# ArtRand/cPecan-signal

Hardware: AMD Instinct MI355X
Metric: banded fwd-bwd Gcells/s (higher is better)
Workload: dtype f64

## Files before the change

cpecan-signal_amd/csrc/asm/gen_sweeps.py:

```python
#!/usr/bin/env python3
import os
import struct
import sys

from emit import Emitter, Neg, Pool, S, V

L = 3
P = 64 * L

LAYER_BYTES = 2 * 64 * 16
OFF_FXY = 64 * 16
OFF_PY = L * LAYER_BYTES
PY2_X2 = os.environ.get("CPECAN_ASM_PY2", "x2") == "x2"
ROW_BYTES = L * LAYER_BYTES + 1024 + (512 if PY2_X2 else 1024)
ROW_DOUBLES = ROW_BYTES // 8
assert L == 3
TRACK_ROW_BYTES = 20 * 8
NCONST = 18

A_ITEMS, A_TRACKBASE, A_PLANWIN, A_PLANCTL, A_PLANOFF, A_EVENTS, A_MODELS, A_TRACK = 0, 8, 16, 24, 32, 40, 48, 56
A_RING, A_RINGDOUBLES, A_STATES, A_CTX, A_CTXBYTES, A_COEF, A_NITEMS, A_WINDOW = 64, 72, 80, 88, 96, 104, 112, 116
A_RINGD, A_MAXWIN, A_SCRATCH, A_SCRATCHBYTES, A_LOGTHR, A_MODELSTRIDE, ARGS_BYTES = 120, 124, 128, 136, 144, 152, 168
A_MASKTAB = 160
I_LX, I_LY, I_YOFF, I_DIAGBASE, I_MODEL, I_RAGGEDL, I_RAGGEDR, ITEM_BYTES = 0, 8, 24, 48, 112, 116, 120, 128
# ... 7 lines not shown
CTX_X = L * 9 * 1024
CTX_S = CTX_X + 2 * L * 1536
CTX_BYTES = CTX_S + 256

LDS_COEF = 0
LDS_EV = 512
EVN = 256
LDS_ROWS = LDS_EV + ((2 * EVN + L) * 16 + 63) // 64 * 64
ROWN = 64
LDS_F_BYTES = LDS_ROWS + ROWN * TRACK_ROW_BYTES
LDS_PX = 512
PXN = 64
LDS_RF = LDS_PX + PXN * 16
LDS_RF_XY_T = LDS_RF
LDS_B_BYTES = LDS_RF + L * 1024

MAX_WIDTH = 158
BLOCK = 64

ABLATE = set(os.environ.get("CPECAN_ASM_ABLATE", "").split())

LOG2E_F32 = 0x3FB8AA3B
LN2_F32 = 0x3F317218


def dbits(x):
    return struct.unpack("<Q", struct.pack("<d", x))[0]


class Kernel(Emitter):
# ... 103 lines not shown
            self.valu("v_fma_f64", dst, dst, "-0.5", K)
        self.pool.give(*t1s)

    def ladd_front_group(self, pairs, free=()):
        p = self.pool
        recs = [[p.take(2), p.take(2), p.take(2), None, None] for _ in pairs]
        for (x, y), r in zip(pairs, recs):
            self.valu("v_max_f64", r[0], x, y)
        for (x, y), r in zip(pairs, recs):
            self.valu("v_min_f64", r[1], x, y)
        p.give(*free)
        for r in recs:
            self.add(r[2], r[0], Neg(r[1]))
        return recs

    def s_mov64_lit(self, dst, value):
        self.salu("s_mov_b32", dst.lo, "0x%x" % (value & 0xFFFFFFFF))
        self.salu("s_mov_b32", dst.hi, "0x%x" % (value >> 32))

    def add64(self, dst, a, b_lo, b_hi=0):
        self.salu("s_add_u32", dst.lo, a.lo, b_lo)
        self.salu("s_addc_u32", dst.hi, a.hi, b_hi)

    def pc_of(self, dst, label):
        here = self.newlabel("pc")
        self.salu("s_getpc_b64", dst)
        self.label(here)
        self.salu("s_add_u32", dst.lo, dst.lo, "%s-%s" % (label, here))
        self.salu("s_addc_u32", dst.hi, dst.hi, 0)

# ... 58 lines not shown
    sPlanRec = S(90, 2)
    lbl = lambda s: ".L_%s_%s" % (name, s)

    def load_store_masks(q):
        k.salu("s_lshl_b32", sT[0], sD, 6)
        k.salu("s_add_u32", sT[0], sT[0], 32)
        k.smem("s_load_dwordx4", S(sMaskS[q][0].i, 4), sMaskTab, sT[0])
        k.salu("s_add_u32", sT[0], sT[0], 16)
        if PY2_X2:
            k.smem("s_load_dwordx2", sMaskS[q][2], sMaskTab, sT[0])
            k.salu("s_add_u32", sT[0], sT[0], 8)
            k.smem("s_load_dwordx2", sMaskPy2[q], sMaskTab, sT[0])
        else:
            k.smem("s_load_dwordx2", sMaskS[q][2], sMaskTab, sT[0])

    def masked_store(mask, dwords, voff, data, off, gate=None):
        if "NOSTORE" in ABLATE or ("NOSTORE4" in ABLATE and dwords == 4) or ("NOSTORE2" in ABLATE and dwords == 2):
            return
        if "STOREALL" in ABLATE:
            if gate is None:
                k.gstore(dwords, voff, data, sRow0 if off < 4096 else sRow1, off % 4096)
            return
        if isinstance(mask, tuple):
            k.salu("s_or_b64", "exec", mask[0], mask[1])
        elif gate is None:
            k.salu("s_mov_b64", "exec", mask)
        else:
            k.salu("s_and_b64", "exec", mask, gate)
        if "EXECONLY" not in ABLATE:
            k.gstore(dwords, voff, data, sRow0 if off < 4096 else sRow1, off % 4096)
        k.salu("s_mov_b64", "exec", -1)
# ... 183 lines not shown
        k.salu("s_sub_u32", sD, sD, 1)
        k.lgkm = []
        k.salu("s_bitcmp1_b64", sStepMin, sD)
        if "NOEVENTS" not in ABLATE:
            k.branch("s_cbranch_scc1", lbl("leave%d" % p))
        k.label(lbl("left%d" % p))
        k.salu("s_bitcmp1_b64", sStepMax, sD)
        if "NOEVENTS" not in ABLATE:
            k.branch("s_cbranch_scc1", lbl("enter%d" % p))
        k.label(lbl("entered%d" % p))
        k.lgkm = pend
        k.salu("s_and_b32", sT[0], sD, sRingMask)
        k.salu("s_mul_i32", sT[0], sT[0], ROW_BYTES)
        k.add64(sRow0, sRing, sT[0])
        k.add64(sRow1, sRow0, 4096)

        def lower(j, w):
            return (Xm(q, j - 1), Xx(q, j - 1))[w] if j else R[q].sub(2 * w, 2)

        def middle(j, w):
            return (Xm(p, j - 1), Xx(p, j - 1), Xy(p, j - 1))[w] if j else R[p].sub(2 * w, 2)

        if "HALFPRIO" in ABLATE:
            k.salu("s_setprio", 2)
        aa, bb = [pool.take(2) for _ in range(L)], [pool.take(2) for _ in range(L)]
        for j in range(L):
            k.add(aa[j], lower(j, 0), C[j][CPXO])
        for j in range(L):
            k.add(bb[j], lower(j, 1), C[j][CPXE])
        recs = k.ladd_front_group(list(zip(aa, bb)), free=aa + bb)
# ... 61 lines not shown
        k.need_recs(recs)
        k.ladd_back_group(recs, [Xy(p, j) for j in range(L)])
        k.salu("s_bitcmp1_b64", sFull, sD)
        k.branch("s_cbranch_scc1", lbl("full%d" % p))
        k.label(lbl("fulled%d" % p))
        recs = k.ladd_front_group([(Xm(p, j), csum[j]) for j in range(L)], free=csum)
        k.ladd_rows(recs)
        k.ror64(R[p].sub(2, 2), Xx(p, L - 1))
        k.ror64(R[p].sub(4, 2), Xy(p, L - 1))
        k.need_recs(recs)
        k.ladd_back_group(recs, [Xm(p, j) for j in range(L)])
        masked_store(sMaskS[p][0], 4, vOff16, V(Xm(p, 0).i, 4), 0)
        k.ror64(R[p].sub(0, 2), Xm(p, L - 1))
        for j in range(1, L):
            masked_store(sMaskS[p][j], 4, vOff16, V(Xm(p, j).i, 4), j * LAYER_BYTES)
        k.salu("s_add_u32", sD, sD, 1)

    k.label(lbl("even"))
    step(0)
    state_after = list(k.lgkm)
    k.salu("s_cmp_gt_i32", sD, sTop)
    k.branch("s_cbranch_scc1", lbl("done"))
    k.label(lbl("odd"))
    k.vm = []
    step(1)
    k.salu("s_cmp_le_i32", sD, sStop)
    k.branch("s_cbranch_scc1", lbl("even"))
    k.salu("s_cmp_gt_i32", sD, sTop)
    k.branch("s_cbranch_scc1", lbl("done"))
    k.salu("s_swappc_b64", sRet, sStagePC)
    k.branch("s_branch", lbl("even"))

    for p in range(2):
        k.forget()
        k.label(lbl("full%d" % p))
        for j in range(L):
            masked_store(sMaskS[p][j], 4, vOff16, V(X[p][j].i + 4, 4), j * LAYER_BYTES + OFF_FXY)
        k.branch("s_branch", lbl("fulled%d" % p))
    for p in range(2):
        k.forget()
        k.label(lbl("leave%d" % p))
        k.salu("s_add_u32", sXmin, sXmin, 1)
        k.salu("s_lshl_b64", sBit, 1, sOutL)
        for j in range(L - 1):
            k.salu("s_cmp_eq_u32", sOutJ, j)
            k.branch("s_cbranch_scc1", lbl("leave%d_%d" % (p, j)))
        for j in reversed(range(L)):
            if j < L - 1:
                k.label(lbl("leave%d_%d" % (p, j)))
            k.salu("s_andn2_b64", sMask[j], sMask[j], sBit)
# ... 327 lines not shown
    sRow0, sRow1 = S(20, 2), S(22, 2)
    SM = [S(24 + 8 * q, 8) for q in range(3)]
    def SMm(q, j): return SM[q].sub(2 * j, 2)
    def SMxmin(q): return SM[q].sub(6)
    def SMxmax(q): return SM[q].sub(7)
    sB = [S(24 + i) for i in range(24)]
    def sBp(i): return S(24 + i, 2)
    sMaskTab, sTrack = S(48, 2), S(50, 2)
    sTMM, sTXM, sTYM, sTMY, sTYY = S(52, 2), S(54, 2), S(56, 2), S(58, 2), S(60, 2)
    s7p5, sNinf = S(62, 2), S(64, 2)
    sRf, sWtot, sCandKx, sCandFb, sState = S(66, 2), S(68, 2), S(70, 2), S(72, 2), S(74, 2)
    sA = [S(76 + i) for i in range(16)]
    def sAp(i): return S(76 + i, 2)
    sRet, sStagePC = S(92, 2), S(94, 2)
    sLm = [S(96 + 2 * j, 2) for j in range(L)]
    sCmp = [S(84 + 2 * j, 2) for j in range(L)]
    lbl = lambda s: ".L_%s_%s" % (name, s)

    k.label(name)
    if "PRIOB" in ABLATE:
        k.salu("s_setprio", 2)
    k.smem("s_load_dwordx4", S(24, 4), sArg, A_NITEMS)
    k.smem("s_load_dwordx2", sBp(4), sArg, A_PLANWIN)
    k.smem("s_load_dwordx2", sBp(6), sArg, A_STATES)
    k.smem("s_load_dwordx2", sBp(8), sArg, A_ITEMS)
    k.smem("s_load_dwordx2", sBp(10), sArg, A_LOGTHR)
    k.wait_lgkm()
    k.salu("s_cmp_ge_u32", sWg, sB[0])
    k.branch("s_cbranch_scc1", lbl("exit"))
    k.salu("s_mov_b32", sWindow, sB[1])
# ... 132 lines not shown
    k.salu("s_mov_b32", sNTot, 0)
    k.salu("s_mov_b32", sTd, sTop)
    k.valu("v_mov_b32_e32", vThr.lo, 0)
    k.valu("v_mov_b32_e32", vThr.hi, "0x7ff00000")
    k.salu("s_sub_u32", sRefCnt, sTop, sTpost0)
    k.salu("s_cmp_le_i32", sTop, sFrom)
    k.branch("s_cbranch_scc0", lbl("nodecode"))
    k.valu("v_mov_b32_e32", vThr.lo, vCthr.lo)
    k.valu("v_mov_b32_e32", vThr.hi, vCthr.hi)
    k.label(lbl("nodecode"))
    k.pc_of(sStagePC, lbl("stage"))
    k.wait_all()
    for h in range(2):
        k.rol64(RP.sub(2 * h, 2), PX[0].sub(2 * h, 2))
    def prefetch_terms(dreg, masks=None):
        k.salu("s_and_b32", sA[0], dreg, sRingMask)
        k.salu("s_mul_i32", sA[0], sA[0], ROW_BYTES)
        k.add64(sAp(4), sRing0, sA[0])
        for j in range(L):
            if masks is not None:
                k.salu("s_lshr_b64", sAp(8), masks[j], 8)
                k.salu("s_lshl_b64", sAp(10), masks[j], 56)
                k.salu("s_or_b64", sAp(8), sAp(8), sAp(10))
                k.salu("s_or_b64", "exec", sAp(8), masks[j])
            k.add64(sAp(2), sAp(4), j * LAYER_BYTES + OFF_FXY)
            k.salu("s_mov_b32", "m0", LDS_RF_XY_T + j * 1024)
            k.nop(1)
            k.gload_lds(vOff16, sAp(2))
        if masks is not None:
            k.salu("s_mov_b64", "exec", -1)

    prefetch_terms(sTpost0)
    k.salu("s_mul_hi_u32", sA[0], sTop, "0x55555556")
    k.salu("s_mul_i32", sA[0], sA[0], 3)
    k.salu("s_sub_u32", sA[0], sTop, sA[0])
    k.salu("s_cmp_eq_u32", sA[0], 1)
    k.branch("s_cbranch_scc1", lbl("entry1"))
    k.salu("s_cmp_eq_u32", sA[0], 2)
    k.branch("s_cbranch_scc1", lbl("entry2"))

    def row_bases(dreg):
        k.salu("s_and_b32", sA[0], dreg, sRingMask)
        k.salu("s_mul_i32", sA[0], sA[0], ROW_BYTES)
        k.add64(sRow0, sRing0, sA[0])
        k.add64(sRow1, sRing1, sA[0])

    def fetch_row(q, masks):
        for j in range(L):
            k.salu("s_mov_b64", "exec", masks[j])
            off = j * LAYER_BYTES
            k.gload(4, T[q][j], vOff16, sRow0 if off < 4096 else sRow1, off % 4096)
            if j:
                if j == 1:
                    k.salu("s_or_b64", "exec", masks[0], masks[1])
                off = OFF_PY + (j - 1) * 1024
                if j == 2 and PY2_X2:
                    k.salu("s_mov_b64", "exec", sLmPy2)
                    k.gload(2, PYB4[q][1], vOff8, sRow0 if off < 4096 else sRow1, off % 4096)
                else:
                    k.gload(4, PYB4[q][j - 1], vOff16, sRow0 if off < 4096 else sRow1, off % 4096)
        k.salu("s_mov_b64", "exec", -1)

    def load_masks(q, dreg):
        k.salu("s_max_i32", sA[0], dreg, 0)
        k.salu("s_lshl_b32", sA[0], sA[0], 6)
        k.smem("s_load_dwordx8", SM[q], sMaskTab, sA[0])

    def load_row_masks(dreg):
        k.salu("s_max_i32", sA[0], dreg, 0)
        k.salu("s_lshl_b32", sA[0], sA[0], 6)
        k.salu("s_add_u32", sA[0], sA[0], 32)
        k.smem("s_load_dwordx4", S(96, 4), sMaskTab, sA[0])
        k.salu("s_add_u32", sA[0], sA[0], 16)
        k.smem("s_load_dwordx2", S(100, 2), sMaskTab, sA[0])
        if PY2_X2:
            k.salu("s_add_u32", sA[0], sA[0], 8)
            k.smem("s_load_dwordx2", sLmPy2, sMaskTab, sA[0])

    for kk in (0, 1, 2):
        k1, k2 = (kk + 1) % 3, (kk + 2) % 3
        k.forget()
        k.label(lbl("entry%d" % kk))
        load_masks(kk, sTd)
        k.salu("s_sub_u32", sA[1], sTd, 1)
        load_masks(k2, sA[1])
        k.salu("s_sub_u32", sA[1], sTd, 2)
        load_masks(k1, sA[1])
        load_row_masks(sTd)
        k.drain_lgkm()
        for j in range(L):
            k.salu("s_mov_b64", "exec", SMm(kk, j))
            for dst, src in ((M[kk][j], e[0]), (BX[j], e[1]), (BY[j], e[2])):
# ... 23 lines not shown
def backward_loop(k, v):
    g = dict(v)
    k.mods = " nt" if "NT" in ABLATE or "NTB" in ABLATE else ""
    name, pool, lbl = g["name"], g["pool"], g["lbl"]
    M, BX, BY, UM, UY, T, PYB, PX, RP = g["M"], g["BX"], g["BY"], g["UM"], g["UY"], g["T"], g["PYB"], g["PX"], g["RP"]
    PMB, PYB4, sLmPy2, FBS = g["PMB"], g["PYB4"], g["sLmPy2"], g["FBS"]
    Tf, Tpm, PXo, PXe = g["Tf"], g["Tpm"], g["PXo"], g["PXe"]
    vOff16, vOff8, vTmp, vTmp2, vThr, vCthr = g["vOff16"], g["vOff8"], g["vTmp"], g["vTmp2"], g["vThr"], g["vCthr"]
    SM, SMm, SMxmin, SMxmax, sLm, sA, sAp = g["SM"], g["SMm"], g["SMxmin"], g["SMxmax"], g["sLm"], g["sA"], g["sAp"]
    sTd, sTo, sFrom, sTop, sTpost0, sNCand, sNTot, sCandCap, sRefCnt, sStop = \
        g["sTd"], g["sTo"], g["sFrom"], g["sTop"], g["sTpost0"], g["sNCand"], g["sNTot"], g["sCandCap"], g["sRefCnt"], g["sStop"]
    sTMM, sTXM, sTYM, sTMY, sTYY, s7p5, sNinf = g["sTMM"], g["sTXM"], g["sTYM"], g["sTMY"], g["sTYY"], g["s7p5"], g["sNinf"]
    sRow0, sRow1, sRf, sWtot, sCandKx, sCandFb, sState = g["sRow0"], g["sRow1"], g["sRf"], g["sWtot"], g["sCandKx"], g["sCandFb"], g["sState"]
    sRet, sStagePC, sTrack, sWindow, sMaskTab = g["sRet"], g["sStagePC"], g["sTrack"], g["sWindow"], g["sMaskTab"]
    row_bases, fetch_row, load_masks, load_row_masks, sCmp = g["row_bases"], g["fetch_row"], g["load_masks"], g["load_row_masks"], g["sCmp"]
    prefetch_terms, sRingMask, sRing0 = g["prefetch_terms"], g["sRingMask"], g["sRing0"]
    sNxt = S(90, 2)

    for kk in (0, 1, 2):
        k1, k2 = (kk + 1) % 3, (kk + 2) % 3
        k.forget()
        k.label(lbl("head%d" % kk))
        k.drain_lgkm()
        rhB, rhP, rBx = pool.take(2), pool.take(2), pool.take(2)
        k.rol64(rhB, M[k2][0])
        k.rol64(rhP, PMB[k2][0])
        k.rol64(rBx, BX[0])
        sB_ = [M[k2][j + 1] if j < L - 1 else rhB for j in range(L)]
        sP_ = [PMB[k2][j + 1] if j < L - 1 else rhP for j in range(L)]
        sBx_ = [BX[j + 1] if j < L - 1 else rBx for j in range(L)]
# ... 12 lines not shown
                k.add(dst[j], sB_[j], dst[j])
        pool.give(rhB, rhP, rBx)
        k.salu("s_cmp_lg_u64", SM[k1].sub(6, 2), SM[kk].sub(6, 2))
        if "NOEVENTS" not in ABLATE:
            k.branch("s_cbranch_scc1", lbl("band%d" % kk))
        k.label(lbl("banded%d" % kk))
        k.salu("s_mov_b64", sNxt, SM[k1].sub(6, 2))
        k.salu("s_sub_u32", sA[1], sTd, 2)
        if "NOMASKB" not in ABLATE:
            load_masks(k1, sA[1])
        k.salu("s_sub_u32", sA[1], sTd, 2)
        row_bases(sA[1])
        ra = k.ladd_front_group([(bmin[j], UM[j]) for j in range(L)], free=bmin)
        rb = k.ladd_front_group([(byin[j], UY[j]) for j in range(L)], free=byin)
        k.ladd_rows(ra + rb)
        for j in range(L):
            k.salu("s_mov_b64", "exec", sLm[j])
            off = j * LAYER_BYTES
            if "NOLOAD" not in ABLATE:
                k.gload(4, T[k1][j], vOff16, sRow0 if off < 4096 else sRow1, off % 4096)
                if j and "NOPY" not in ABLATE:
                    if j == 1:
                        k.salu("s_or_b64", "exec", sLm[0], sLm[1])
                    off = OFF_PY + (j - 1) * 1024
                    if j == 2 and PY2_X2:
                        k.salu("s_mov_b64", "exec", sLmPy2)
                        k.gload(2, PYB4[k1][1], vOff8, sRow0 if off < 4096 else sRow1, off % 4096)
                    else:
                        k.gload(4, PYB4[k1][j - 1], vOff16, sRow0 if off < 4096 else sRow1, off % 4096)
            k.salu("s_mov_b64", "exec", -1)
        k.salu("s_sub_u32", sA[1], sTd, 3)
        if "NOMASKB" not in ABLATE:
            load_row_masks(sA[1])
        k.need_recs(ra)
        k.ladd_back_group(ra, [M[kk][j] for j in range(L)])
        rc = k.ladd_front_group([(bxin[j], y1[j]) for j in range(L)], free=bxin + y1)
        k.ladd_rows(rc)
        k.need_recs(rb)
        k.ladd_back_group(rb, BY)
        rd = k.ladd_front_group([(M[kk][j], y2[j]) for j in range(L)], free=y2)
        k.ladd_rows(rd)
        k.need_recs(rc)
        k.ladd_back_group(rc, BX)
        k.need_recs(rd)
        k.ladd_back_group(rd, [M[kk][j] for j in range(L)])
# ... 319 lines not shown
    nv = (k.pool.first + 2 * k.pool.high + 7) // 8 * 8
    kernels.append(dict(name=name, body=k.text(), lds=LDS_B_BYTES, kernarg=ARGS_BYTES, vgprs=nv, sgprs=102, accum=nv,
                        stats=dict(k.stats, vgprs=nv)))
    text = ['\t.amdgcn_target "amdgcn-amd-amdhsa--gfx950"', "\t.amdhsa_code_object_version 6"]
    for kk in kernels:
        text.append(KERNEL_TEMPLATE.format(**kk))
    text.append("\t.amdgpu_metadata\n---\namdhsa.kernels:")
    for kk in kernels:
        text.append(META_TEMPLATE.format(**kk).rstrip("\n"))
    text.append("amdhsa.target:   amdgcn-amd-amdhsa--gfx950\namdhsa.version:\n  - 1\n  - 2\n...\n\n\t.end_amdgpu_metadata")
    open(out, "w").write("\n".join(text) + "\n")
    if len(sys.argv) > 2:
        defs = dict(ASM_L=L, ASM_ROW_BYTES=ROW_BYTES, ASM_LAYER_BYTES=LAYER_BYTES, ASM_OFF_FXY=OFF_FXY, ASM_OFF_PY=OFF_PY, ASM_PY2_X2=int(PY2_X2), ASM_CTX_X=CTX_X, ASM_CTX_S=CTX_S, ASM_CTX_BYTES=CTX_BYTES,
                    ASM_MAX_WIDTH=MAX_WIDTH, ASM_PLANWIN_BYTES=PLANWIN_BYTES, ASM_CTL_BYTES=CTL_BYTES, ASM_BLOCK=BLOCK,
                    ASM_ARGS_BYTES=ARGS_BYTES, ASM_NCONST=NCONST, ASM_MASK_BYTES=MASK_BYTES, ASM_MASK_GROUP=MASK_GROUP, ASM_LDS_F_BYTES=LDS_F_BYTES, ASM_LDS_B_BYTES=LDS_B_BYTES)
        with open(sys.argv[2], "w") as h:
            h.write("/* generated by asm/gen_sweeps.py: what the assembly sweeps and the C++ side agree on */\n")
            h.write("#ifndef CPECAN_ASM_GEN_H_\n#define CPECAN_ASM_GEN_H_\n")
            for kname, val in defs.items():
                h.write("#define %s %d\n" % (kname, val))
            h.write("#endif\n")
    for kk in kernels:
        sys.stderr.write("%s: %s\n" % (kk["name"], kk["stats"]))


if __name__ == "__main__":
    main()
```

cpecan-signal_amd/csrc/cpecan_asm.hip:

```cpp
#include "cpecan_asm.h"

#include <algorithm>
#include <mutex>

namespace {

const unsigned char SWEEPS_HSACO[] = {
#include "cpecan_sweeps_hsaco.inc"
};

struct PerDevice {
    bool tried = false, ok = false;
    hipModule_t module = nullptr;
    hipFunction_t forward = nullptr, backward = nullptr;
    double *coef = nullptr;
};
std::mutex g_lock;
PerDevice g_dev[64];

void fill_coef(double *c) {
    const float t[16] = { -0.009350833524763f, 0.130659527668286f, 0.498799810682272f, 0.693203116424741f,
                          -0.014532321752540f, 0.139942324101744f, 0.495635523139337f, 0.692140569840976f,
                          -0.004605031767994f, 0.063427417320019f, 0.695956496475118f, 0.514272634594009f,
                          -0.000458661602210f, 0.009695946122598f, 0.930734667215156f, 0.168037164329057f };
// ... 71 lines not shown
        }
    if (lane < 16) {
        const int s[16] = { 1, 0, 0, 0, 0, 0, 1 / ASM_L, 1 % ASM_L, 0, 0, 0, 0, 0, 0, 0, 0 };
        ((int *) (c + ASM_CTX_S))[lane] = s[lane];
    }
    double *r = ring + idx * ringDoubles + (long long) ringD * (ASM_ROW_BYTES / 8);
    for (int i = lane; i < ASM_ROW_BYTES / 8; i += 64) r[i] = ninf;
}

extern "C" __global__ void cpecan_k_asm_masks(const DevItem *items, long long nItems, const int *bandTab, unsigned *maskTab) {
    for (long long idx = blockIdx.y; idx < nItems; idx += gridDim.y) {
        const DevItem it = items[idx];
        const long long d = (long long) blockIdx.x * blockDim.x + threadIdx.x;
        if (d > it.lX + it.lY) continue;
        const int lo = bandTab[2 * (it.diagBase + d)], hi = bandTab[2 * (it.diagBase + d) + 1];
        unsigned long long m[ASM_L], g[ASM_L];
        for (int j = 0; j < ASM_L; j++) m[j] = g[j] = 0ull;
        for (int x = lo - 1; x <= hi + 1; x++) {
            const int s = (x + 64 * ASM_L) % (64 * ASM_L);
            g[s % ASM_L] |= ((1ull << ASM_MASK_GROUP) - 1) << ((s / ASM_L) & ~(ASM_MASK_GROUP - 1));
            if (x >= lo && x <= hi) m[s % ASM_L] |= 1ull << (s / ASM_L);
        }
        unsigned *e = maskTab + (it.diagBase + d) * (ASM_MASK_BYTES / 4);
        for (int j = 0; j < ASM_L; j++) {
            e[2 * j] = (unsigned) m[j];
            e[2 * j + 1] = (unsigned) (m[j] >> 32);
            e[8 + 2 * j] = (unsigned) g[j];
            e[9 + 2 * j] = (unsigned) (g[j] >> 32);
        }
        e[6] = (unsigned) lo;
        e[7] = (unsigned) hi;
        unsigned long long h = 0ull;
        for (int q = 0; q < 64; q += 16)
            if (g[ASM_L - 1] & (0xFFFFull << q)) h |= 0xFFFFull << q;
        e[14] = (unsigned) h;
        e[15] = (unsigned) (h >> 32);
    }
}

extern "C" hipError_t cpecan_asm_launch_masks(hipStream_t stream, const DevItem *items, long long nItems, long long maxDiags,
                                              const int *bandTab, unsigned *maskTab) {
    hipLaunchKernelGGL(cpecan_k_asm_masks, dim3((unsigned) ((maxDiags + 255) / 256), (unsigned) std::min(nItems, 65535LL)),
                       dim3(256), 0, stream, items, nItems, bandTab, maskTab);
    return hipGetLastError();
}

extern "C" __global__ void cpecan_k_asm_begin(const DevItem *items, long long nItems, double *ring, long long ringDoubles) {
    const long long idx = (long long) blockIdx.x * blockDim.x + threadIdx.x;
    if (idx >= nItems) return;
    const DevItem it = items[idx];
    double *r = ring + idx * ringDoubles;
    r[0] = it.raggedL ? CP_NEG_INF : 0.0;
    r[1] = 0.0;
    r[ASM_OFF_PY / 8] = 0.0;
    r[ASM_OFF_FXY / 8] = r[ASM_OFF_FXY / 8 + 1] = it.raggedL ? 0.0 : CP_NEG_INF;
}

extern "C" hipError_t cpecan_asm_launch_ctx_init(hipStream_t stream, const DevItem *items, long long nItems, char *ctx,
                                                 long long ctxBytes, double *ring, long long ringDoubles, int ringD) {
    hipLaunchKernelGGL(cpecan_k_asm_ctx_init, dim3((unsigned) nItems), dim3(64), 0, stream, items, nItems, ctx, ctxBytes,
                       ring, ringDoubles, ringD);
    return hipGetLastError();
}

extern "C" int cpecan_asm_launch_begin(hipStream_t stream, const DevItem *items, long long nItems, double *ring,
                                       long long ringDoubles) {
// ... 5 lines not shown
```

cpecan-signal_amd/csrc/cpecan_asm_gen.h:

```cpp
#ifndef CPECAN_ASM_GEN_H_
#define CPECAN_ASM_GEN_H_
#define ASM_L 3
#define ASM_ROW_BYTES 7680
#define ASM_LAYER_BYTES 2048
#define ASM_OFF_FXY 1024
#define ASM_OFF_PY 6144
#define ASM_PY2_X2 1
#define ASM_CTX_X 27648
#define ASM_CTX_S 36864
#define ASM_CTX_BYTES 37120
#define ASM_MAX_WIDTH 158
#define ASM_PLANWIN_BYTES 64
#define ASM_CTL_BYTES 32
#define ASM_BLOCK 64
#define ASM_ARGS_BYTES 168
#define ASM_NCONST 18
#define ASM_MASK_BYTES 64
#define ASM_MASK_GROUP 8
#define ASM_LDS_F_BYTES 19008
#define ASM_LDS_B_BYTES 4608
#endif
```

cpecan-signal_amd/csrc/cpecan_device.h:

```cpp
#ifndef CPECAN_DEVICE_H_
#define CPECAN_DEVICE_H_

#include <hip/hip_runtime.h>
#include <stdint.h>

#define CP_NEG_INF (-__builtin_huge_val())

#define CP_ROW 18
#define CP_MU 0
#define CP_SD 1
#define CP_RSD 2
#define CP_K1 3
#define CP_NMU 4
#define CP_NSD 5
#define CP_RNSD 6
#define CP_K2 7
#define CP_YMU 8
#define CP_YSD 9
#define CP_RYSD 10
#define CP_YK1 11
#define CP_YNMU 12
#define CP_YNSD 13
#define CP_RYNSD 14
#define CP_YK2 15
// ... 40 lines not shown
    long long nCells;
    long long pairBase, pairCap;
    long long totBase, totCap;
    long long bwsBase;
    int model, raggedL, raggedR, maxWidth;
};

struct DevParams {
    double threshold;
    long long minDiags, tbDiags, expansion;
    int mode, debug, unbanded;
    int scanDecode;
    double logThrSlack;
    int ldsWidth;
    int expectResweep;
};

struct DevGeneralArgs {
    const DevItem *items;
    const int *bandL, *bandR;
    const long long *cellPrefix;
    const void *x;
    const void *y;
    const double *yAux;
    const void *models;
    double *F, *B;
    long long *pairs;
    double *pairLogp;
    long long *nPairs, *totXay;
    double *totVal;
    long long *nTot;
// ... 61 lines not shown
```

cpecan-signal_amd/csrc/cpecan_hip.hip:

```cpp
#include "cpecan_hip.h"

#include "cpecan_device.h"
#include "cpecan_asm.h"
#include "cpecan_sweep.h"

#include <hip/hip_runtime.h>

#include <algorithm>
#include <array>
#include <atomic>
#include <chrono>
#include <climits>
#include <cmath>
#include <cstdarg>
#include <cstdio>
#include <cstring>
#include <mutex>
#include <new>
#include <string>
#include <sched.h>
#include <thread>
#include <vector>

extern "C" __global__ void cpecan_k_general(DevGeneralArgs, DevParams);
// ... 1631 lines not shown
    b->maxWidth = plan.maxWidth;
    b->compactPairs = plan.maxLXY + m.xReach < 65536;
    b->nModels = m.nModels(c);
    b->expectLen = m.expectLen;
    b->P.threshold = bp.threshold;
    b->P.minDiags = bp.minDiagsBetweenTraceBack;
    b->P.tbDiags = bp.traceBackDiagonals;
    b->P.expansion = bp.diagonalExpansion;
    b->P.mode = in.mode;
    b->P.debug = (d.flags & CPECAN_FLAG_DEBUG_DUMP) ? 1 : 0;
    b->P.unbanded = in.unbanded ? 1 : 0;
    b->P.scanDecode = (d.flags & CPECAN_FLAG_SCAN_DECODE) ? 1 : 0;
    b->P.logThrSlack = bp.threshold > 0.0 ? log(bp.threshold) - 1e-3 : -INFINITY;
    b->P.ldsWidth = 0;
    b->P.expectResweep = 0;
    if (d.build) {
        b->sy = d.build;
        b->trackRow = b->sy->once->trackRowDoubles;
    }
    b->hItems = plan.items;
    return b;
}


static int upload_sequences(cpecan_batch *b, const BatchInput &in) {
    cpecan_ctx *c = b->ctx;
    const MachineRow &m = MACHINES[b->machine];
    const int64_t nItems = in.nItems, nX = in.nX, nEvents = in.nEvents;
    B_TRY(b->items.alloc((size_t) nItems));
    B_TRY(hipMemcpyAsync(b->items.p, b->hItems.data(), (size_t) nItems * sizeof(DevItem), hipMemcpyHostToDevice, c->prep));
// ... 384 lines not shown
    all.kidx = b->kidx.p; all.kid = b->kid.p; all.Fring = b->Fstore.p; all.ringDoubles = b->ringDoubles;
    all.ringD = b->ringD; all.states = b->syStates.p; all.stateBytes = b->stateBytes; all.pairs = b->pairs.p;
    all.pairLogp = b->pairLogp.p; all.totXay = b->totXay.p; all.totVal = b->totVal.p; all.scratch = b->syScratch.p;
    all.scratchBytes = b->scratchBytes; all.Bring = b->Bring.p; all.bringRow = sy->bringRowDoubles;
    all.expect = b->expect.p; all.nPairs = b->nPairs.p; all.nTot = b->nTot.p; all.nCells = b->nCells.p;
    all.models = (const double *) MACHINES[b->machine].models(c);
    if (sy->machine == SWEEP_HDP) {
        for (const DevHdpModel &m : c->hostModelsH)
            if (m.t[T_GAP_SWITCH_TO_X] > -INFINITY) all.withSwitch = 1;
    } else if (sy->machine == SWEEP_STRAWMAN) {
        for (int m = 0; m < c->nModels; m++)
            if (c->switchToX[(size_t) m] > -INFINITY) all.withSwitch = 1;
    }
    int rc = sy->once->launch_track(L->fwd, all);
    const bool asmRun = b->useAsm && !all.withSwitch && rc == 0;
    AsmArgs asmArgs{};
    if (asmRun) {
        asmArgs.items = b->items.p; asmArgs.trackBase = b->trackBase.p; asmArgs.planWin = b->planWin.p;
        asmArgs.planCtl = b->planCtl.p; asmArgs.planOff = b->planOff.p; asmArgs.events = b->events.p;
        asmArgs.models = c->models.p; asmArgs.track = b->track.p; asmArgs.ring = b->Fstore.p;
        asmArgs.ringDoubles = b->ringDoubles; asmArgs.states = b->syStates.p; asmArgs.ctx = b->asmCtx.p;
        asmArgs.ctxBytes = ASM_CTX_BYTES; asmArgs.coef = cpecan_asm_coef(c->device); asmArgs.nItems = (int) b->nItems;
        asmArgs.ringD = b->ringD; asmArgs.maxWindows = b->asmMaxWindows; asmArgs.scratch = b->syScratch.p;
        asmArgs.scratchBytes = b->scratchBytes; asmArgs.logThrSlack = b->P.logThrSlack; asmArgs.modelStride = CP_MODEL_STRIDE;
        asmArgs.maskTab = b->asmMasks.p;
        rc = cpecan_asm_launch_begin(L->fwd, b->items.p, b->nItems, b->Fstore.p, b->ringDoubles);
        if (getenv("CPECAN_ASM_TRACE")) {
            auto span = [](const char *what, const void *p, size_t bytes) {
                fprintf(stderr, "[cpecan asm]   %-10s %p .. %p (%zu bytes)\n", what, p, (const char *) p + bytes, bytes);
            };
// ... 631 lines not shown
```

cpecan-signal_amd/csrc/cpecan_kernel_wave.hip:

```cpp
#include "cpecan_device.h"
#include "cpecan_sweep.h"

#include <vector>

#ifndef WV_L
#define WV_L 3
#endif
#define WV_P (64 * WV_L)
#if defined(WV_VANILLA) && WV_L == 4
#define WV_SYM(n) n##_v4
#elif defined(WV_VANILLA) && WV_L == 3
#define WV_SYM(n) n##_v3
#elif defined(WV_VANILLA)
#define WV_SYM(n) n##_v2
#elif defined(WV_HDP) && WV_L == 4
#define WV_SYM(n) n##_h4
#elif defined(WV_HDP) && WV_L == 3
#define WV_SYM(n) n##_h3
#elif defined(WV_HDP)
#define WV_SYM(n) n##_h2
#elif WV_L == 4
#define WV_SYM(n) n##_l4
#elif WV_L == 3
#define WV_SYM(n) n##_l3
// ... 1018 lines not shown
                    mask_clear(fm, 1ull << topL, topJ);
                    topJ = uni(topJ - 1);
                    if (topJ < 0) { topJ = L - 1; topL = uni((topL + 63) & 63); }
                }
                if ((fwMin >> bi) & 1u) {
                    ev |= 2u | (unsigned) botL << 10 | (unsigned) botJ << 16 | (unsigned) ((fxmin - 1) & (WV_PXN - 1)) << 18;
                    mask_set(fm, 1ull << botL, botJ);
                    fxmin--;
                    botJ = uni(botJ - 1);
                    if (botJ < 0) { botJ = L - 1; botL = uni((botL + 63) & 63); }
                }
            }
            r.ev = ev;
            const bool live = FX ? tau >= tracedBackTo : tau > tracedBackTo;
            const unsigned rowOff = (unsigned) ((long long) (tau & ringMask) * (WV_ROW_DOUBLES * 8));
#pragma unroll
            for (int j = 0; j < L; j++) {
                r.m[j] = live ? fm[j] : 0ull;
                unsigned offA, offB;
                const unsigned realA = rowOff + voffA[j], dummyA = dummyOff + voffA[j];
                const unsigned realB = rowOff + voffB[j], dummyB = dummyOff + voffB[j];
                asm("v_cndmask_b32 %0, %1, %2, %3" : "=v"(offA) : "v"(dummyA), "v"(realA), "s"(r.m[j]));
                asm("v_cndmask_b32 %0, %1, %2, %3" : "=v"(offB) : "v"(dummyB), "v"(realB), "s"(r.m[j]));
                const d2 fp = *(const d2 *) ((const char *) ring + offA);
                q.f[j] = fp.x;
                q.pm[j] = fp.y;
                q.py[j] = *(const double *) ((const char *) ring + offB);
                if (FX) {
                    const d2 fxy = *(const d2 *) ((const char *) ring + offA + (WV_OFF_FX(0) - WV_OFF_FM(0)) * 8);
                    q.fx[j] = fxy.x;
                    q.fy[j] = fxy.y;
                }
            }
        };

        Rec r0, r1;
// ... 358 lines not shown
            const int sl = lane * L + j, sMinN = nmn % WV_P;
            return nmn + (sl - sMinN + (sl < sMinN ? WV_P : 0));
        };
#endif
        auto flags = [&](const int i, const int j, bool &tv, bool &nv, bool &below) __attribute__((always_inline)) {
            const int xmn = uni(sh.rec[i][1]), xmx = uni(sh.rec[i][2]), nmn = uni(sh.rec[i][3]), nmx = uni(sh.rec[i][4]);
            const bool second = uni(sh.rec[i][5]) != 0;
            const int pxmin = uni(sh.rec[i][6]), pxmax = uni(sh.rec[i][7]);
            const int sl = lane * L + j, sMin = xmn % WV_P, sMinN = nmn % WV_P;
            const int xT = xmn + (sl - sMin + (sl < sMin ? WV_P : 0));
            const int xN = nmn + (sl - sMinN + (sl < sMinN ? WV_P : 0));
            tv = xT <= xmx;
            nv = second && xN <= nmx;
            below = nv && xN - 1 >= pxmin && xN - 1 <= pxmax;
        };
        auto issue = [&](const int i, Ops (&o)[L]) __attribute__((always_inline)) {
            const int t = uni(sh.rec[i][0]);
            const double *rowT = ring + (long long) (t & ringMask) * WV_ROW_DOUBLES;
            const double *rowB = ring + (long long) ((t - 1) & ringMask) * WV_ROW_DOUBLES;
            const double *src = rf + (long long) (base + i) * (5 * WV_P) + lane;
#pragma unroll
            for (int j = 0; j < L; j++) {
                bool tv, nv, below;
                flags(i, j, tv, nv, below);
                const int sl = lane * L + j, sb = sl == 0 ? WV_P - 1 : sl - 1;
                const double *pa = rowT + (tv ? j : 0) * WV_LAYER_DOUBLES;
                const double *pb = rowB + (below ? sb % L : 0) * WV_LAYER_DOUBLES;
                const int la = tv ? lane : 0, lb = below ? sb / L : 0;
                o[j].fm = pa[WV_OFF_FM(la)]; o[j].fx = pa[WV_OFF_FX(la)]; o[j].fy = pa[WV_OFF_FY(la)];
                o[j].s0 = pb[WV_OFF_FM(lb)]; o[j].s1 = pb[WV_OFF_FX(lb)]; o[j].s2 = pb[WV_OFF_FY(lb)];
                o[j].bm = src[(0 * L + j) * 64];
                o[j].bx = src[(1 * L + j) * 64];
                o[j].by = src[(2 * L + j) * 64];
                o[j].hb = src[(3 * L + j) * 64];
                o[j].hp = src[(4 * L + j) * 64];
#ifdef WV_VANILLA
                const double *tr = track + (long long) (nv ? column_above(i, j) : 0) * WV_ROW;
                o[j].tm = tr[18];
                o[j].tx = tr[19];
#endif
            }
        };
        auto work = [&](const int i, const Ops (&o)[L]) __attribute__((always_inline)) {
// ... 902 lines not shown
```

Before: 67.18.

## Store ring rows band-relative so live cells pack contiguously from lane0

Adds a band-rotated row layout: each diagonal row in the ring buffer is stored with position computed relative to the lane of the band's lower x bound, so valid cells occupy a contiguous run of slots. Store and load offsets in the assembly sweeps, the mask builder, the ring init, and the HIP wave kernel readers are all rotated accordingly. Mask groups are rebuilt as contiguous runs. The aim is to make masked global stores and loads touch fewer, denser cache lines, at the cost of extra scalar/vector offset arithmetic and an extra scalar load plus lgkm drain in prefetch.

```diff
diff --git a/cpecan-signal_amd/csrc/asm/gen_sweeps.py b/cpecan-signal_amd/csrc/asm/gen_sweeps.py
--- a/cpecan-signal_amd/csrc/asm/gen_sweeps.py
+++ b/cpecan-signal_amd/csrc/asm/gen_sweeps.py
@@ -45,6 +45,8 @@
 LDS_RF = LDS_PX + PXN * 16
 LDS_RF_XY_T = LDS_RF
 LDS_B_BYTES = LDS_RF + L * 1024
+
+ROWS_BAND = os.environ.get("CPECAN_ASM_ROWS", "lane") == "band"
 
 MAX_WIDTH = 158
 BLOCK = 64
@@ -178,6 +180,20 @@
             self.add(r[2], r[0], Neg(r[1]))
         return recs
 
+    def row_offsets(self, v16, v8, vOff16, s16):
+        self.valu("v_subrev_u32_e32", v16, s16, vOff16)
+        self.valu("v_and_b32_e32", v16, "0x3f0", v16)
+        if v8 is not None:
+            self.valu("v_lshrrev_b32_e32", v8, 1, v16)
+
+    def lane0_of_xmin(self, dst, tmp, xmin):
+        self.salu("s_add_u32", dst, xmin, P - 1)
+        self.salu("s_mul_hi_u32", tmp, dst, "0x%x" % ((1 << 32) // P + 1))
+        self.salu("s_mul_i32", tmp, tmp, P)
+        self.salu("s_sub_u32", dst, dst, tmp)
+        self.salu("s_mul_hi_u32", dst, dst, "0x%x" % ((1 << 32) // L + 1))
+        self.salu("s_lshl_b32", dst, dst, 4)
+
     def s_mov64_lit(self, dst, value):
         self.salu("s_mov_b32", dst.lo, "0x%x" % (value & 0xFFFFFFFF))
         self.salu("s_mov_b32", dst.hi, "0x%x" % (value >> 32))
@@ -266,7 +282,11 @@
         else:
             k.smem("s_load_dwordx2", sMaskS[q][2], sMaskTab, sT[0])
 
+    rot = {}
+
     def masked_store(mask, dwords, voff, data, off, gate=None):
+        if ROWS_BAND:
+            voff = rot["cur"][0 if voff is vOff16 else 1]
         if "NOSTORE" in ABLATE or ("NOSTORE4" in ABLATE and dwords == 4) or ("NOSTORE2" in ABLATE and dwords == 2):
             return
         if "STOREALL" in ABLATE:
@@ -480,6 +500,14 @@
         k.salu("s_mul_i32", sT[0], sT[0], ROW_BYTES)
         k.add64(sRow0, sRing, sT[0])
         k.add64(sRow1, sRow0, 4096)
+        if ROWS_BAND:
+            tr = pool.take(2)
+            rot[p] = rot["cur"] = (tr.lo, tr.hi)
+            k.salu("s_cmp_eq_u32", sOutJ, 0)
+            k.salu("s_cselect_b32", sT[1], 16, 0)
+            k.salu("s_lshl_b32", sT[2], sOutL, 4)
+            k.salu("s_sub_u32", sT[1], sT[2], sT[1])
+            k.row_offsets(rot[p][0], rot[p][1], vOff16, sT[1])
 
         def lower(j, w):
             return (Xm(q, j - 1), Xx(q, j - 1))[w] if j else R[q].sub(2 * w, 2)
@@ -571,6 +599,8 @@
         k.ror64(R[p].sub(0, 2), Xm(p, L - 1))
         for j in range(1, L):
             masked_store(sMaskS[p][j], 4, vOff16, V(Xm(p, j).i, 4), j * LAYER_BYTES)
+        if ROWS_BAND:
+            pool.give(V(rot[p][0].i, 2))
         k.salu("s_add_u32", sD, sD, 1)
 
     k.label(lbl("even"))
@@ -591,6 +621,7 @@
     for p in range(2):
         k.forget()
         k.label(lbl("full%d" % p))
+        rot["cur"] = rot.get(p)
         for j in range(L):
             masked_store(sMaskS[p][j], 4, vOff16, V(X[p][j].i + 4, 4), j * LAYER_BYTES + OFF_FXY)
         k.branch("s_branch", lbl("fulled%d" % p))
@@ -948,6 +979,7 @@
     def sAp(i): return S(76 + i, 2)
     sRet, sStagePC = S(92, 2), S(94, 2)
     sLm = [S(96 + 2 * j, 2) for j in range(L)]
+    sLmX = sA[7]
     sCmp = [S(84 + 2 * j, 2) for j in range(L)]
     lbl = lambda s: ".L_%s_%s" % (name, s)
 
@@ -1110,6 +1142,16 @@
     for h in range(2):
         k.rol64(RP.sub(2 * h, 2), PX[0].sub(2 * h, 2))
     def prefetch_terms(dreg, masks=None):
+        vo = vOff16
+        if ROWS_BAND:
+            k.salu("s_max_i32", sA[0], dreg, 0)
+            k.salu("s_lshl_b32", sA[0], sA[0], 6)
+            k.salu("s_add_u32", sA[0], sA[0], 24)
+            k.smem("s_load_dword", sA[1], sMaskTab, sA[0])
+            k.drain_lgkm()
+            k.lane0_of_xmin(sA[1], sA[0], sA[1])
+            vo = pool.take(1)
+            k.row_offsets(vo, None, vOff16, sA[1])
         k.salu("s_and_b32", sA[0], dreg, sRingMask)
         k.salu("s_mul_i32", sA[0], sA[0], ROW_BYTES)
         k.add64(sAp(4), sRing0, sA[0])
@@ -1122,9 +1164,11 @@
             k.add64(sAp(2), sAp(4), j * LAYER_BYTES + OFF_FXY)
             k.salu("s_mov_b32", "m0", LDS_RF_XY_T + j * 1024)
             k.nop(1)
-            k.gload_lds(vOff16, sAp(2))
+            k.gload_lds(vo, sAp(2))
         if masks is not None:
             k.salu("s_mov_b64", "exec", -1)
+        if ROWS_BAND:
+            pool.give(vo)
 
     prefetch_terms(sTpost0)
     k.salu("s_mul_hi_u32", sA[0], sTop, "0x55555556")
@@ -1141,7 +1185,19 @@
         k.add64(sRow0, sRing0, sA[0])
         k.add64(sRow1, sRing1, sA[0])
 
+    def row_rot():
+        if not ROWS_BAND:
+            return vOff16, vOff8
+        tr = pool.take(2)
+        v16, v8 = tr.lo, tr.hi
+        k.lane0_of_xmin(sA[0], sA[1], sLmX)
+        k.row_offsets(v16, v8, vOff16, sA[0])
+        return v16, v8
+
     def fetch_row(q, masks):
+        vOff16, vOff8 = row_rot()
+        if ROWS_BAND:
+            pool.give(V(vOff16.i, 2))
         for j in range(L):
             k.salu("s_mov_b64", "exec", masks[j])
             off = j * LAYER_BYTES
@@ -1172,6 +1228,9 @@
         if PY2_X2:
             k.salu("s_add_u32", sA[0], sA[0], 8)
             k.smem("s_load_dwordx2", sLmPy2, sMaskTab, sA[0])
+        if ROWS_BAND:
+            k.salu("s_sub_u32", sA[0], sA[0], 32 if PY2_X2 else 24)
+            k.smem("s_load_dword", sLmX, sMaskTab, sA[0])
 
     for kk in (0, 1, 2):
         k1, k2 = (kk + 1) % 3, (kk + 2) % 3
@@ -1225,6 +1284,7 @@
     sRow0, sRow1, sRf, sWtot, sCandKx, sCandFb, sState = g["sRow0"], g["sRow1"], g["sRf"], g["sWtot"], g["sCandKx"], g["sCandFb"], g["sState"]
     sRet, sStagePC, sTrack, sWindow, sMaskTab = g["sRet"], g["sStagePC"], g["sTrack"], g["sWindow"], g["sMaskTab"]
     row_bases, fetch_row, load_masks, load_row_masks, sCmp = g["row_bases"], g["fetch_row"], g["load_masks"], g["load_row_masks"], g["sCmp"]
+    row_rot = g["row_rot"]
     prefetch_terms, sRingMask, sRing0 = g["prefetch_terms"], g["sRingMask"], g["sRing0"]
     sNxt = S(90, 2)
 
@@ -1267,6 +1327,7 @@
         ra = k.ladd_front_group([(bmin[j], UM[j]) for j in range(L)], free=bmin)
         rb = k.ladd_front_group([(byin[j], UY[j]) for j in range(L)], free=byin)
         k.ladd_rows(ra + rb)
+        vOff16, vOff8 = row_rot()
         for j in range(L):
             k.salu("s_mov_b64", "exec", sLm[j])
             off = j * LAYER_BYTES
@@ -1282,6 +1343,9 @@
                     else:
                         k.gload(4, PYB4[k1][j - 1], vOff16, sRow0 if off < 4096 else sRow1, off % 4096)
             k.salu("s_mov_b64", "exec", -1)
+        if ROWS_BAND:
+            pool.give(V(vOff16.i, 2))
+            vOff16, vOff8 = g["vOff16"], g["vOff8"]
         k.salu("s_sub_u32", sA[1], sTd, 3)
         if "NOMASKB" not in ABLATE:
             load_row_masks(sA[1])
@@ -1631,6 +1695,8 @@
         defs = dict(ASM_L=L, ASM_ROW_BYTES=ROW_BYTES, ASM_LAYER_BYTES=LAYER_BYTES, ASM_OFF_FXY=OFF_FXY, ASM_OFF_PY=OFF_PY, ASM_PY2_X2=int(PY2_X2), ASM_CTX_X=CTX_X, ASM_CTX_S=CTX_S, ASM_CTX_BYTES=CTX_BYTES,
                     ASM_MAX_WIDTH=MAX_WIDTH, ASM_PLANWIN_BYTES=PLANWIN_BYTES, ASM_CTL_BYTES=CTL_BYTES, ASM_BLOCK=BLOCK,
                     ASM_ARGS_BYTES=ARGS_BYTES, ASM_NCONST=NCONST, ASM_MASK_BYTES=MASK_BYTES, ASM_MASK_GROUP=MASK_GROUP, ASM_LDS_F_BYTES=LDS_F_BYTES, ASM_LDS_B_BYTES=LDS_B_BYTES)
+        if ROWS_BAND:
+            defs["ASM_ROWS_BAND"] = 1
         with open(sys.argv[2], "w") as h:
             h.write("/* generated by asm/gen_sweeps.py: what the assembly sweeps and the C++ side agree on */\n")
             h.write("#ifndef CPECAN_ASM_GEN_H_\n#define CPECAN_ASM_GEN_H_\n")
diff --git a/cpecan-signal_amd/csrc/cpecan_asm.hip b/cpecan-signal_amd/csrc/cpecan_asm.hip
--- a/cpecan-signal_amd/csrc/cpecan_asm.hip
+++ b/cpecan-signal_amd/csrc/cpecan_asm.hip
@@ -109,13 +109,33 @@
         const long long d = (long long) blockIdx.x * blockDim.x + threadIdx.x;
         if (d > it.lX + it.lY) continue;
         const int lo = bandTab[2 * (it.diagBase + d)], hi = bandTab[2 * (it.diagBase + d) + 1];
-        unsigned long long m[ASM_L], g[ASM_L];
+        unsigned long long m[ASM_L], g[ASM_L], h = 0ull;
         for (int j = 0; j < ASM_L; j++) m[j] = g[j] = 0ull;
+#ifdef ASM_ROWS_BAND
+        int n[ASM_L];
+        for (int j = 0; j < ASM_L; j++) n[j] = 0;
+#endif
         for (int x = lo - 1; x <= hi + 1; x++) {
             const int s = (x + 64 * ASM_L) % (64 * ASM_L);
+#ifdef ASM_ROWS_BAND
+            n[s % ASM_L] = ring_pos(s / ASM_L, lo, ASM_L) + 1;
+#else
             g[s % ASM_L] |= ((1ull << ASM_MASK_GROUP) - 1) << ((s / ASM_L) & ~(ASM_MASK_GROUP - 1));
+#endif
             if (x >= lo && x <= hi) m[s % ASM_L] |= 1ull << (s / ASM_L);
         }
+#ifdef ASM_ROWS_BAND
+        const int lane0 = ((lo + 64 * ASM_L - 1) % (64 * ASM_L)) / ASM_L;
+        auto run = [lane0](int cnt) {
+            const unsigned long long ones = cnt >= 64 ? ~0ull : (1ull << cnt) - 1;
+            return lane0 ? (ones << lane0) | (ones >> (64 - lane0)) : ones;
+        };
+        for (int j = 0; j < ASM_L; j++) g[j] = run((n[j] + ASM_MASK_GROUP - 1) / ASM_MASK_GROUP * ASM_MASK_GROUP);
+        h = run((n[ASM_L - 1] + 15) / 16 * 16);
+#else
+        for (int q = 0; q < 64; q += 16)
+            if (g[ASM_L - 1] & (0xFFFFull << q)) h |= 0xFFFFull << q;
+#endif
         unsigned *e = maskTab + (it.diagBase + d) * (ASM_MASK_BYTES / 4);
         for (int j = 0; j < ASM_L; j++) {
             e[2 * j] = (unsigned) m[j];
@@ -125,9 +145,6 @@
         }
         e[6] = (unsigned) lo;
         e[7] = (unsigned) hi;
-        unsigned long long h = 0ull;
-        for (int q = 0; q < 64; q += 16)
-            if (g[ASM_L - 1] & (0xFFFFull << q)) h |= 0xFFFFull << q;
         e[14] = (unsigned) h;
         e[15] = (unsigned) (h >> 32);
     }
@@ -145,6 +162,9 @@
     if (idx >= nItems) return;
     const DevItem it = items[idx];
     double *r = ring + idx * ringDoubles;
+#ifdef ASM_ROWS_BAND
+    r += 2 * ring_pos(0, 0, ASM_L);
+#endif
     r[0] = it.raggedL ? CP_NEG_INF : 0.0;
     r[1] = 0.0;
     r[ASM_OFF_PY / 8] = 0.0;
diff --git a/cpecan-signal_amd/csrc/cpecan_asm_gen.h b/cpecan-signal_amd/csrc/cpecan_asm_gen.h
--- a/cpecan-signal_amd/csrc/cpecan_asm_gen.h
+++ b/cpecan-signal_amd/csrc/cpecan_asm_gen.h
@@ -19,4 +19,5 @@
 #define ASM_MASK_GROUP 8
 #define ASM_LDS_F_BYTES 19008
 #define ASM_LDS_B_BYTES 4608
+#define ASM_ROWS_BAND 1
 #endif
diff --git a/cpecan-signal_amd/csrc/cpecan_device.h b/cpecan-signal_amd/csrc/cpecan_device.h
--- a/cpecan-signal_amd/csrc/cpecan_device.h
+++ b/cpecan-signal_amd/csrc/cpecan_device.h
@@ -78,7 +78,13 @@
     double logThrSlack;
     int ldsWidth;
     int expectResweep;
+    int rowsBand;
 };
+
+__host__ __device__ inline int ring_pos(int lane, int xminD, int L) {
+    const int lane0 = ((xminD + 64 * L - 1) % (64 * L)) / L;
+    return (lane - lane0) & 63;
+}
 
 struct DevGeneralArgs {
     const DevItem *items;
diff --git a/cpecan-signal_amd/csrc/cpecan_hip.hip b/cpecan-signal_amd/csrc/cpecan_hip.hip
--- a/cpecan-signal_amd/csrc/cpecan_hip.hip
+++ b/cpecan-signal_amd/csrc/cpecan_hip.hip
@@ -1669,6 +1669,7 @@
     b->P.logThrSlack = bp.threshold > 0.0 ? log(bp.threshold) - 1e-3 : -INFINITY;
     b->P.ldsWidth = 0;
     b->P.expectResweep = 0;
+    b->P.rowsBand = 0;
     if (d.build) {
         b->sy = d.build;
         b->trackRow = b->sy->once->trackRowDoubles;
@@ -2083,6 +2084,9 @@
     }
     int rc = sy->once->launch_track(L->fwd, all);
     const bool asmRun = b->useAsm && !all.withSwitch && rc == 0;
+#ifdef ASM_ROWS_BAND
+    all.P.rowsBand = asmRun ? 1 : 0;
+#endif
     AsmArgs asmArgs{};
     if (asmRun) {
         asmArgs.items = b->items.p; asmArgs.trackBase = b->trackBase.p; asmArgs.planWin = b->planWin.p;
diff --git a/cpecan-signal_amd/csrc/cpecan_kernel_wave.hip b/cpecan-signal_amd/csrc/cpecan_kernel_wave.hip
--- a/cpecan-signal_amd/csrc/cpecan_kernel_wave.hip
+++ b/cpecan-signal_amd/csrc/cpecan_kernel_wave.hip
@@ -1056,12 +1056,14 @@
             r.ev = ev;
             const bool live = FX ? tau >= tracedBackTo : tau > tracedBackTo;
             const unsigned rowOff = (unsigned) ((long long) (tau & ringMask) * (WV_ROW_DOUBLES * 8));
+            const int rot = P.rowsBand ? ring_pos(lane, fxmin, L) - lane : 0;
 #pragma unroll
             for (int j = 0; j < L; j++) {
                 r.m[j] = live ? fm[j] : 0ull;
                 unsigned offA, offB;
-                const unsigned realA = rowOff + voffA[j], dummyA = dummyOff + voffA[j];
-                const unsigned realB = rowOff + voffB[j], dummyB = dummyOff + voffB[j];
+                const unsigned rotA = (unsigned) (rot * 16), rotB = (unsigned) (rot * (((L & 1) && j == L - 1) ? 8 : 16));
+                const unsigned realA = rowOff + voffA[j] + rotA, dummyA = dummyOff + voffA[j];
+                const unsigned realB = rowOff + voffB[j] + rotB, dummyB = dummyOff + voffB[j];
                 asm("v_cndmask_b32 %0, %1, %2, %3" : "=v"(offA) : "v"(dummyA), "v"(realA), "s"(r.m[j]));
                 asm("v_cndmask_b32 %0, %1, %2, %3" : "=v"(offB) : "v"(dummyB), "v"(realB), "s"(r.m[j]));
                 const d2 fp = *(const d2 *) ((const char *) ring + offA);
@@ -1450,6 +1452,7 @@
             nv = second && xN <= nmx;
             below = nv && xN - 1 >= pxmin && xN - 1 <= pxmax;
         };
+        auto xmn_of = [&](const int i) __attribute__((always_inline)) { return uni(sh.rec[i][1]); };
         auto issue = [&](const int i, Ops (&o)[L]) __attribute__((always_inline)) {
             const int t = uni(sh.rec[i][0]);
             const double *rowT = ring + (long long) (t & ringMask) * WV_ROW_DOUBLES;
@@ -1462,7 +1465,11 @@
                 const int sl = lane * L + j, sb = sl == 0 ? WV_P - 1 : sl - 1;
                 const double *pa = rowT + (tv ? j : 0) * WV_LAYER_DOUBLES;
                 const double *pb = rowB + (below ? sb % L : 0) * WV_LAYER_DOUBLES;
-                const int la = tv ? lane : 0, lb = below ? sb / L : 0;
+                int la = tv ? lane : 0, lb = below ? sb / L : 0;
+                if (P.rowsBand) {
+                    la = tv ? ring_pos(lane, xmn_of(i), L) : 0;
+                    lb = below ? ring_pos(sb / L, uni(sh.rec[i][6]), L) : 0;
+                }
                 o[j].fm = pa[WV_OFF_FM(la)]; o[j].fx = pa[WV_OFF_FX(la)]; o[j].fy = pa[WV_OFF_FY(la)];
                 o[j].s0 = pb[WV_OFF_FM(lb)]; o[j].s1 = pb[WV_OFF_FX(lb)]; o[j].s2 = pb[WV_OFF_FY(lb)];
                 o[j].bm = src[(0 * L + j) * 64];
```

Measured after the change: 66.39. -1.2%, worse.
